# smithlabcode/epievo

Measured on AMD Instinct MI355X. Metric: site-branch path resamples/sec at n=1e6, 4-leaf tree, higher is better.
Workload: dtype f64

## Files before the change

epievo_amd/csrc/epv_abi.hip:

```cpp
#include <hip/hip_runtime.h>

#include <algorithm>
#include <chrono>
#include <cmath>
#include <cstdio>
#include <cstdlib>
#include <cstring>
#include <string>
#include <new>
#include <vector>

#include "epievo_mi355x.h"
#include "epv_device.h"
#include "epv_plan.h"

#define EPV_API extern "C" __attribute__((visibility("default")))

#include "epv_kernels.h"
#include "epv_math.h"
#include "epv_pavg.h"
#include "epv_bevents.h"
#include "epv_mixing.h"
#include "epv_wstat.h"
#include "epv_epochs.h"
// ... 1508 lines not shown
  auto raise = [](int kib, auto... kernels) {
    ((void)hipFuncSetAttribute(reinterpret_cast<const void *>(kernels), hipFuncAttributeMaxDynamicSharedMemorySize, kib * 1024), ...);
  };
  raise(128, p3_kernel(1u), p3_kernel(2u), p3_leaf_kernel(1u), p3_leaf_kernel(2u));
  raise(160, p2_kernel(false), p2_kernel(true), p2_leaf_kernel(false), p2_leaf_kernel(true));
  for (uint32_t nn = 0; nn <= EPV_P2_SMALL_MAX; ++nn) raise(160, fused_kernel(nn, false), fused_kernel(nn, true), fused_leaf_kernel(nn));
  for (int v = 0; v < 4; ++v)
    raise(160, v1_kernel<>(v & 1, v & 2), v1_kernel<leaf_arg_t>(v & 1, v & 2), v1_kernel<leaf_arg_t, leaf_arg_t>(v & 1, v & 2));
}

struct PhaseArgs {
  uint32_t colour, seed_lo, seed_hi, sweep;
  uint64_t first, last, own_lo, own_hi;
  uint64_t s0;
  uint64_t threads, blocks;
};

int launch_fused(epv_ctx *c, const PhasePlan &P, const PhaseArgs &a) {
  const PlanV2 &v = c->shapes.v2;
  const int frc = ensure_fused_buffers(c);
  if (frc) return frc;
  const unsigned pb = (unsigned)((a.threads + v.fused_lanes - 1u) / v.fused_lanes);
  if (pb > c->fused_waves) return fail(c, EPV_ERR_STATE, "fused phase: launch larger than its lists");
  EpvFused F = c->F;
  F.meta_cache = P.meta_cache ? 1u : 0u;
  F.lanes = v.fused_lanes;
  F.grouped_rounds = 4u;
  F.topo = 0u;
  for (uint32_t node = 1; node < P.small_nn; ++node)
    F.topo |= (c->subtree[node] == 1u ? 1u << node : 0u) | (c->parent[node] << (8u + 3u * node));
  F.giveups = c->d_counters + EPV_CNT_WORDS;
  if (P.unobs || P.evidence)
    hipLaunchKernelGGL(fused_leaf_kernel(P.small_nn), dim3(pb), dim3(64), v.lds, c->stream, c->S, a.colour, a.seed_lo,
                       a.seed_hi, a.sweep, a.first, a.last, a.own_lo, a.own_hi, v.pool, 0u, 0u, c->d_counters, (double *)nullptr,
                       c->d_segtab, F, (leaf_arg_t)c->d_evidence, (leaf_arg_t)c->d_unobs);
  else
  hipLaunchKernelGGL(fused_kernel(P.small_nn, P.direct), dim3(pb), dim3(64), v.lds, c->stream, c->S, a.colour, a.seed_lo,
                     a.seed_hi, a.sweep, a.first, a.last, a.own_lo, a.own_hi, v.pool, 0u, 0u, c->d_counters, (double *)nullptr,
                     c->d_segtab, F);
  return EPV_OK;
}

template <class... Leaf>
void launch_v1(epv_ctx *c, const PhasePlan &P, const PhaseArgs &a, Leaf... leaf) {
  const PlanV1 &v = c->shapes.v1;
  hipLaunchKernelGGL(v1_kernel<Leaf...>(P.gpool, P.refq), dim3((unsigned)a.blocks), dim3(v.threads), v.lds, c->stream, c->S,
                     a.colour, a.seed_lo, a.seed_hi, a.sweep, a.first, a.last, v.pool_entries, c->d_counters,
                     P.gpool ? c->d_gpool : (double *)nullptr, leaf...);
}
int launch_propose(epv_ctx *c, const PhasePlan &P, const PhaseArgs &a, uint32_t list_mode) {
  if (P.propose == EPV_PLAN_V3) {
    const PlanV3 &v = c->shapes.v3;
    const int rc = ensure_slab(c, &c->d_gpool3, &c->gpool3_cap, v.slab_need);
    if (rc) return rc;
    if (P.unobs || P.evidence)
      hipLaunchKernelGGL(p3_leaf_kernel(P.p3_words), dim3((unsigned)((a.threads + 255u) / 256u)), dim3(256), v.lds, c->stream,
                         c->S, a.colour, a.seed_lo, a.seed_hi, a.sweep, a.first, a.last, a.own_lo, a.own_hi, v.list_cap, v.qrows,
                         v.n_up, v.depth, list_mode - 1u, c->d_counters, c->d_gpool3, c->d_segtab, c->d_nodetab, c->d_slabflags,
                         v.slots, (leaf_arg_t)c->d_evidence, (leaf_arg_t)c->d_unobs);
    else
    hipLaunchKernelGGL(p3_kernel(P.p3_words), dim3((unsigned)((a.threads + 255u) / 256u)), dim3(256), v.lds, c->stream, c->S,
                       a.colour, a.seed_lo, a.seed_hi, a.sweep, a.first, a.last, a.own_lo, a.own_hi, v.list_cap, v.qrows,
                       v.n_up, v.depth, list_mode - 1u, c->d_counters, c->d_gpool3, c->d_segtab, c->d_nodetab, c->d_slabflags,
                       v.slots);
    ++c->phase_parity;
  } else if (P.propose == EPV_PLAN_V2) {
    const PlanV2 &v = c->shapes.v2;
    const bool seg = P.jumps == EPV_PLAN_JUMPS_SEGMENTS;
    if (seg) { const int rc = ensure_seg_buffers(c); if (rc) return rc; }
    if (P.unobs || P.evidence)
      hipLaunchKernelGGL(p2_leaf_kernel(seg), dim3((unsigned)((a.threads + 63u) / 64u)), dim3(64), v.lds, c->stream, c->S,
                         a.colour, a.seed_lo, a.seed_hi, a.sweep, a.first, a.last, a.own_lo, a.own_hi, v.pool, 0u, list_mode - 1u,
                         c->d_counters, (double *)nullptr, c->d_segtab, EpvFused{}, (leaf_arg_t)c->d_evidence,
                         (leaf_arg_t)c->d_unobs);
    else
    hipLaunchKernelGGL(p2_kernel(seg), dim3((unsigned)((a.threads + 63u) / 64u)), dim3(64), v.lds, c->stream, c->S, a.colour,
                       a.seed_lo, a.seed_hi, a.sweep, a.first, a.last, a.own_lo, a.own_hi, v.pool, 0u, list_mode - 1u,
                       c->d_counters, (double *)nullptr, c->d_segtab, EpvFused{});
    ++c->phase_parity;
  } else {
    if (P.gpool) { const int rc = ensure_slab(c, &c->d_gpool, &c->gpool_cap, c->shapes.v1.slab_need); if (rc) return rc; }
    if (P.evidence) launch_v1(c, P, a, (leaf_arg_t)c->d_evidence, (leaf_arg_t)c->d_unobs);
    else if (P.unobs) launch_v1(c, P, a, (leaf_arg_t)c->d_unobs);
    else launch_v1(c, P, a);
  }
  return EPV_OK;
}

void launch_jumps(epv_ctx *c, const PhasePlan &P, const PhaseArgs &a) {
  const size_t lds = const_lds_bytes(c->S.N);
  unsigned long long *giveups = c->d_counters + EPV_CNT_WORDS;
// ... 1624 lines not shown

EPV_API int epv_get_counters(epv_ctx *c, epv_counters *out) {
  if (!c || !out) return EPV_ERR_ARG;
  HIP_TRY(c, hipSetDevice(c->device));
  unsigned long long cnt[EPV_CNT_N];
  int rc = read_counters(c, cnt);
  if (rc) return rc;
  out->n_overflow = cnt[EPV_CNT_OVERFLOW];
  out->n_coop_tasks = cnt[EPV_CNT_COOP];
  out->n_sweeps = c->n_sweeps;
  out->n_search_finished = cnt[EPV_CNT_SEARCH_FINISHED];
  return EPV_OK;
}

#ifdef EPV_P2_PROFILE
EPV_API int epv_debug_p2_profile(unsigned long long *out) {
  std::vector<unsigned long long> rows(16u * EPV_P2_PROF_ROWS);
  if (hipMemcpyFromSymbol(rows.data(), HIP_SYMBOL(epv_p2_prof), rows.size() * sizeof(unsigned long long)) != hipSuccess) return 1;
  for (int q = 0; q < 16; ++q) out[q] = 0;
  for (size_t r = 0; r < EPV_P2_PROF_ROWS; ++r)
    for (int q = 0; q < 16; ++q) out[q] += rows[16u * r + q];
  return 0;
}
#endif

EPV_API int epv_set_timing(epv_ctx *c, int enabled) {
  if (!c) return EPV_ERR_ARG;
  c->timing_every = enabled > 0 ? (uint32_t)enabled : 0u;
  c->timing_seen = 0;
  c->timing = false;
  return EPV_OK;
}

EPV_API int epv_kernel_time_ms(epv_ctx *c, double *avg_ms, uint64_t *n_launches) {
  if (!c || !avg_ms || !n_launches) return EPV_ERR_ARG;
  HIP_TRY(c, hipSetDevice(c->device));
  HIP_TRY(c, hipStreamSynchronize(c->stream));
  int rc = drain_timing(c);
  if (rc) return rc;
  *n_launches = c->timed_launches;
  *avg_ms = c->timed_launches ? c->timed_ms / (double)c->timed_launches : 0.0;
  c->timed_ms = 0.0;
  c->timed_launches = 0;
  return EPV_OK;
}

// ... 842 lines not shown
```

epievo_amd/csrc/epv_plan.h:

```cpp
#ifndef EPV_PLAN_H
#define EPV_PLAN_H

#include <algorithm>
#include <cmath>
#include <cstdlib>
#include <vector>

#include "epv_device.h"

struct EpvKnobs {
  bool propose_v1 = false;
  int propose_v3 = -1;
  int seg_jumps = -1;
  int fused_phase = -1;
  bool small_tree = true;
  uint32_t fused_lanes = 0;
  bool force_lds_pool = false, force_global_pool = false;
  bool p3_min_list = false;
  int p3_slab_pool = 1;
  int accept_v3 = -1;
  bool accept_no_cache = false;
};

template <class Lookup>
// ... 70 lines not shown
  const uint32_t N = in.N, B = N - 1u, C = in.C;
  const uint64_t worst = (uint64_t)B * (2u * C + 2u);
  const size_t fixed = const_lds_bytes(N) + (((size_t)N * 64u * 4u + 15u) & ~(size_t)15u);
  if (fixed > 150u * 1024u) return false;
  const uint64_t typical = (uint64_t)(64.0 * B * (2.0 * in.kbar + 2.0) * 1.3) + 32u;
  const uint64_t max_fit = fixed + 16u < 160u * 1024u ? (160u * 1024u - fixed) / 16u : 0u;
  const uint64_t want = std::max<uint64_t>(worst, typical);
  const bool lds_ok = want <= max_fit && (fixed + std::min(want, max_fit) * 16u) * 8u <= 160u * 1024u;
  const bool use_lds = knobs.force_global_pool ? false : knobs.force_lds_pool ? want <= max_fit : lds_ok;
  if (use_lds) {
    const uint64_t pool = std::min(want, max_fit);
    v.pool_entries = (uint32_t)pool;
    v.lds = fixed + (size_t)pool * 16u;
  } else {
    const uint64_t blocks = (epv_phase_cap(in.n_sites) + 63u) / 64u;
    v.slab_need = blocks * worst * 128u;
    v.gpool = true;
    v.pool_entries = (uint32_t)worst;
    v.lds = fixed;
  }
  return true;
}

inline bool plan_p2(const PlanInput &in, const EpvKnobs &knobs, PlanV2 &v) {
  const uint32_t N = in.N, B = N - 1u, C = in.C;
  const uint64_t phase_cap = epv_phase_cap(in.n_sites);
  const size_t shared = const_lds_bytes(N) + (size_t)B * 4u * 6u * 8u;
  const size_t per_wave_fixed = ((((size_t)N * 64u + 1u) / 2u + 1u) & ~(size_t)1u) * 8u +
                                ((3u * 64u + 2u) * (size_t)B * sizeof(epv_meta_t) + 15u) / 16u * 16u;
  const size_t fixed = shared + per_wave_fixed;
  const uint64_t worst_rec = (uint64_t)B * (2u * C + 2u), worst_heavy = (uint64_t)B * (2u * C + 1u);
  uint32_t f_lanes = knobs.fused_lanes ? knobs.fused_lanes : 64u;
  if (!knobs.fused_lanes)
    while (f_lanes > 16u && (phase_cap + f_lanes / 2u - 1u) / (f_lanes / 2u) <= 2048u) f_lanes /= 2u;
  const uint64_t phase_waves = (phase_cap + 63u) / 64u;
  const uint64_t f_bytes = (phase_cap + f_lanes - 1u) / f_lanes *
                           (epv_fused_seg_cap(B, C) * (sizeof(EpvSegTask) + sizeof(EpvSegOut)) + epv_fused_bt_cap(B) * 12u);
  const bool fused = !knobs.propose_v1 && 2u * C + 1u <= 64u && f_bytes <= (4ull << 30) &&
                     (knobs.fused_phase < 0 ? phase_waves <= FUSED_MAX_WAVES : knobs.fused_phase != 0);
  const uint64_t hrec = (fused || seg_jumps_on(knobs, in.kbar)) ? EPV_HREC : EPV_HREC_SHORT;
  const uint64_t worst_dbl = 2u * worst_rec + hrec * worst_heavy;
  const double lam = 2.0 * in.kbar;
  uint32_t n_internal = 0;
  for (uint32_t node = 1; node < N; ++node) n_internal += in.subtree[node] != 1u;
  const double rec_per_lane = B * (1.0 + lam) + n_internal;
  const uint64_t typical_dbl = (uint64_t)(64.0 * (2.0 * rec_per_lane + (double)hrec * B * heavy_per_branch(lam)) * P2_MARGIN) + 64u;
  const uint64_t max_fit = fixed + 64u < 160u * 1024u ? (160u * 1024u - fixed) / 8u : 0u;
  uint64_t want = std::max(worst_dbl, typical_dbl);
  if (fused) want = std::max<uint64_t>(want, std::max<uint64_t>(EPV_COOP_BYTES / 8u, 992u + 48u * (uint64_t)B));
  const bool lds_ok = want <= max_fit && (fixed + want * 8u) * 5u <= 160u * 1024u;
  const bool use_lds = knobs.force_global_pool ? false : knobs.force_lds_pool ? want <= max_fit : lds_ok;
  if (fixed > 150u * 1024u) return false;
  v.planned = use_lds;
  v.fused = fused && use_lds;
  v.fused_lanes = f_lanes;
  v.pool = use_lds ? (uint32_t)((want + 1u) & ~(uint64_t)1u) : 0u;
  v.lds = fixed + (size_t)v.pool * 8u;
  return true;
}

inline PlanV3 plan_p3(const PlanInput &in, const EpvKnobs &knobs, const PlanV2 &v2) {
  const uint32_t N = in.N, B = N - 1u, C = in.C;
  if (knobs.propose_v3 == 0 || knobs.propose_v1 || N > 128u || N < 2u) return {};
  if (knobs.propose_v3 < 0 && v2.planned) return {};
// ... 145 lines not shown
```

epievo_amd/csrc/epv_propose2.h:

```cpp
#ifndef EPV_PROPOSE2_H
#define EPV_PROPOSE2_H

struct EpvSegRec {
  double P00, P11;
  double PT00, PT10;
  double nb0, nb1;
  double u_end, u_first;
  double len;
  uint64_t info;
};

EPV_DEV void epv_seg_matrices(double len, double r0, double r1, double out[6]) {
  const double denom = r0 + r1;
  const double h = 1.0 / epv_exp(len * (r0 + r1));
  out[0] = (r0 * h + r1) / denom;
  out[1] = (r0 + r1 * h) / denom;
  const double h2 = epv_exp(-len * (r0 + r1));
  out[2] = gtp(r0, r1, h2, denom, 0u, 0u);
  out[3] = gtp(r0, r1, h2, denom, 1u, 0u);
#if defined(__HIP_DEVICE_COMPILE__)
  out[4] = nojump_bound(len * r0);
  out[5] = nojump_bound(len * r1);
#else
  out[4] = 0.0;
  out[5] = 0.0;
#endif
}

__global__ void epv_segtab_kernel(EpvDev S, double *tab) {
  const uint32_t t = blockIdx.x * blockDim.x + threadIdx.x;
  if (t >= S.B * 4u) return;
  const uint32_t b = t >> 2, li = (t >> 1) & 1u, ri = t & 1u;
  const double *rates = reinterpret_cast<const double *>(S.model);
  const uint32_t trip0 = 4u * li + ri;
// ... 64 lines not shown
  uint32_t grouped_rounds;
  uint32_t topo;
  unsigned long long *giveups;
};

template <bool SEG, bool FUSED, int NN = 0, bool DIRECT = false, class... Leaf>
__global__ __launch_bounds__(256, EPV_PROPOSE2_WAVES) void epv_mh_propose2_kernel(
    EpvDev S, uint32_t colour, uint32_t seed_lo, uint32_t seed_hi, uint32_t sweep, uint64_t first,
    uint64_t last, uint64_t own_first, uint64_t own_last, uint32_t pool_dbl, uint32_t list_cap,
    uint32_t parity, unsigned long long *counters, double *gpool, const double *segtab, EpvFused F, Leaf... leaf_args) {
  constexpr bool LEAF = sizeof...(Leaf) != 0;
  static_assert(sizeof...(Leaf) == (LEAF ? 2u : 0u), "the table and the mask come together");
  [[maybe_unused]] EpvLeafSrc LS{nullptr, nullptr};
  if constexpr (LEAF) { LS.table = epv_first_arg(leaf_args...); LS.mask = epv_second_arg(leaf_args...); }
  static_assert(!FUSED || SEG, "the fused phase emits segments");
  static_assert(!DIRECT || FUSED, "the direct body is the fused phase's");
  static_assert(!LEAF || !DIRECT, "the fused direct bodies have no leaf variant");
  constexpr bool SMALL = NN > 0;
  static_assert(!SMALL || (FUSED && NN >= 2 && NN <= EPV_P2_SMALL_MAX), "the small-tree body is the fused phase's");
  constexpr int NNA = SMALL ? NN : 1;
  constexpr int NBA = SMALL ? NN - 1 : 1;
  const uint32_t NNODE = SMALL ? (uint32_t)NN : S.N;
  extern __shared__ __attribute__((aligned(16))) double s_mem[];
  constexpr uint32_t HREC = SEG ? EPV_HREC : EPV_HREC_SHORT, LEN_AT = HREC - 2u, INFO_AT = HREC - 1u;
#ifdef EPV_P2_PROFILE
  unsigned long long t_acc_[16] = {0, 0, 0, 0, 0, 0, 0, 0, 0, 0, 0, 0, 0, 0, 0, 0};
  unsigned long long t_prev_ = __builtin_readcyclecounter();
#endif
  const uint32_t B = SMALL ? (uint32_t)NN - 1u : S.B;
  const uint32_t const_dbl = (20u + NNODE + 1u) & ~1u;
  const uint32_t tab_dbl = B * 4u * EPV_SEGTAB_DBL;
  const uint32_t regA_dbl = ((NNODE * 64u + 1u) / 2u + 1u) & ~1u;
  const uint32_t mc_dbl = ((3u * 64u + 2u) * B * (uint32_t)sizeof(epv_meta_t) + 15u) / 16u * 2u;
  const uint32_t wave_id = threadIdx.x >> 6;
  const uint32_t my_shard = (blockIdx.x * (blockDim.x >> 6) + wave_id) & (EPV_SHARDS - 1u);
  const uint32_t wave_dbl = regA_dbl + mc_dbl + ((pool_dbl + 1u) & ~1u);
  double *s_const = s_mem;
  double *s_tab = s_mem + const_dbl;
  double *s_wave = s_mem + const_dbl + tab_dbl + (size_t)wave_id * wave_dbl;
  uint32_t *regA = reinterpret_cast<uint32_t *>(s_wave);
  epv_meta_t *s_meta = reinterpret_cast<epv_meta_t *>(s_wave + regA_dbl);
  epv_meta_t *s_edge = s_meta + 3u * B * 64u;
  const int lane = epv_lane();
  double *pool = s_wave + regA_dbl + mc_dbl;
  const uint64_t gfirst = S.g0 + first;
  const uint64_t s0 = first + ((colour + 3u - (uint32_t)(gfirst % 3u)) % 3u);
  const uint32_t lpw = FUSED ? F.lanes : 64u;
// ... 198 lines not shown
      }
      __builtin_amdgcn_fence(__ATOMIC_SEQ_CST, "wavefront");
      __builtin_amdgcn_wave_barrier();
    } else if (run && heavy) {
      uint32_t hcur = hbase;
      for (uint32_t node = 1u; node < NNODE; ++node) {
        const uint32_t b = node - 1u;
        const uint32_t K = (s_meta[(0u * B + b) * 64u + lane] & EPV_NJ_MASK) + (s_meta[(1u * B + b) * 64u + lane] & EPV_NJ_MASK) + 1u;
        if (K < 2u) continue;
        merge_branch((uint32_t)lane, node, hcur, jbaseL, jbaseR);
        hcur += K;
      }
    }
    __builtin_amdgcn_fence(__ATOMIC_SEQ_CST, "wavefront");
    __builtin_amdgcn_wave_barrier();

    P2_MARK(2);
    for (uint32_t i = (uint32_t)lane; i < totH; i += 64u) {
      double *rec = list + (size_t)i * HREC;
      const double len = rec[LEN_AT];
      const uint64_t info = epv_d2u(rec[INFO_AT]);
      const uint32_t trip0 = (uint32_t)info & 7u, owner = (uint32_t)(info >> 3) & 63u;
      const uint32_t node = (uint32_t)(info >> 9) & 4095u, k = (uint32_t)(info >> 21);
      double m[6];
      epv_seg_matrices(len, s_rates[trip0], s_rates[trip0 | 2u], m);
      const epv_block2 blk = epv_keyed_block<!FUSED>(seed_lo, seed_hi, gsite_lane0 + 3u * owner, sweep, node, k, 0u, 0u);
#pragma unroll
      for (int q = 0; q < 6; ++q) rec[q] = m[q];
      rec[6] = blk.d0;
      rec[7] = blk.d1;
    }
    __builtin_amdgcn_fence(__ATOMIC_SEQ_CST, "wavefront");
    __builtin_amdgcn_wave_barrier();

    P2_MARK(3);
    bool ident = true;
    if (run) {
      uint32_t off = need_rec, hcur = hbase + heavy;
#pragma unroll 1
      for (uint32_t node = NNODE - 1u; node >= 1u; --node) {
        const uint32_t b = node - 1u;
        [[maybe_unused]] uint32_t leaf_word = 0u;
        if constexpr (LEAF) {
          if (SMALL ? EPV_TOPO_LEAF(node) != 0u : S.subtree[node] == 1u) leaf_word = epv_leaf_word(LS, node, site);
        }
        const uint32_t mL = s_meta[(0u * B + b) * 64u + lane], mR = s_meta[(1u * B + b) * 64u + lane];
        const uint32_t K = (mL & EPV_NJ_MASK) + (mR & EPV_NJ_MASK) + 1u;
        const uint32_t sub = SMALL ? 2u - EPV_TOPO_LEAF(node) : S.subtree[node];
        off -= K + (LEAF || sub != 1u ? 1u : 0u);
        double n0 = 1.0, n1 = 1.0;
        if (sub == 1u) {
          const uint32_t mM = s_meta[(2u * B + b) * 64u + lane];
          const uint32_t leaf_state = (mM >> EPV_INIT_SHIFT) ^ (mM & 1u);
// ... 26 lines not shown
          const double *t = s_tab + (b * 4u + 2u * (mL >> EPV_INIT_SHIFT) + (mR >> EPV_INIT_SHIFT)) * EPV_SEGTAB_DBL;
          const double P00 = t[0], P11 = t[1];
          const double P01 = 1.0 - P00, P10 = 1.0 - P11;
          double *rec = my + (size_t)off * RS;
          rec[0] = P00 * n0 + P01 * n1;
          rec[1] = P10 * n0 + P11 * n1;
        } else {
          hcur -= K;
          for (uint32_t kk = K; kk-- > 0u;) {
            const double *hr = list + (size_t)(hcur + kk) * HREC;
            const double P00 = hr[0], P11 = hr[1];
            const double P01 = 1.0 - P00, P10 = 1.0 - P11;
            const double a = P00 * n0 + P01 * n1;
            const double c = P10 * n0 + P11 * n1;
            double *rec = my + (size_t)(off + kk) * RS;
            rec[0] = a; rec[1] = c;
            n0 = a; n1 = c;
          }
        }
      }
    }

    P2_MARK(4);
    unsigned long long dirty = 0ull, multi = 0ull, deep = 0ull;
    const uint32_t root_state = run ? (uint32_t)(s_meta[(2u * B) * 64u + lane] >> EPV_INIT_SHIFT) : 0u;
    uint32_t hcur = hbase;
    if constexpr (SMALL) {
      if (run) {
#pragma unroll
        for (int node = 1; node < NNA; ++node) r_node[node] = regA[(uint32_t)node * 64u + lane];
#pragma unroll
        for (int node = 1; node < NNA; ++node) {
          const int b = node - 1;
          const uint32_t K = EPV_RW_K(r_w[b]);
          const uint32_t off = r_node[node];
          uint32_t start_state = root_state;
#pragma unroll
          for (int p = 1; p < node; ++p)
            if (EPV_TOPO_PARENT(node) == (uint32_t)p) start_state = r_node[p] >> 31;
          const bool leaf = EPV_TOPO_LEAF(node);
          const uint32_t mM = EPV_RW_META(r_w[b]);
          uint32_t prev = start_state;
          bool clean = true;
          unsigned long long word = 0ull, w64 = 0ull;
          double pk0 = my[(size_t)off * RS], pk1 = my[(size_t)off * RS + 1u];
          for (uint32_t k = 0; k < K; ++k) {
            const bool last_seg = (k + 1u == K);
            double nxt0, nxt1;
            if (!LEAF && last_seg && leaf) {
              const uint32_t leaf_state = (mM >> EPV_INIT_SHIFT) ^ (mM & 1u);
              nxt0 = leaf_state ? 0.0 : 1.0;
              nxt1 = leaf_state ? 1.0 : 0.0;
            } else {
              nxt0 = my[(size_t)(off + k + 1u) * RS];
              nxt1 = my[(size_t)(off + k + 1u) * RS + 1u];
            }
            double PT0, nb, u_end, u_first;
            if (K == 1u) {
              const double *t = s_tab + ((uint32_t)b * 4u + EPV_RW_TAB(r_w[b])) * EPV_SEGTAB_DBL;
              PT0 = prev ? t[3] : t[2];
              nb = prev ? t[5] : t[4];
              const epv_block2 blk = epv_keyed_block<!FUSED>(seed_lo, seed_hi, gsite, sweep, (uint32_t)node, 0u, 0u, 0u);
              u_end = blk.d0; u_first = blk.d1;
            } else {
              const double *hr = list + (size_t)(hcur + k) * HREC;
              PT0 = prev ? hr[3] : hr[2];
              nb = prev ? hr[5] : hr[4];
              u_end = hr[6]; u_first = hr[7];
            }
            const double p0 = PT0 * nxt0 / (prev ? pk1 : pk0);
            const uint32_t sampled = (u_end > p0) ? 1u : 0u;
            const bool seg_clean = (sampled == prev) && (1.0 - u_first < nb);
            clean = clean && seg_clean;
            word |= (unsigned long long)sampled << (k & 63u);
            if (k < 64u) w64 = word;
            prev = sampled;
            pk0 = nxt0; pk1 = nxt1;
          }
          const uint32_t hrec0 = hcur;
          if (K >= 2u) hcur += K;
          r_node[node] = off | (prev << 31) | (clean ? 0u : 1u << 30) | (K >= 2u ? hrec0 << 14 : 0u);
          regA[node * 64u + lane] = r_node[node];
          if (!clean && K >= 2u) list[(size_t)hrec0 * HREC + 6u] = epv_u2d(w64);
          s_meta[(2u * B + (uint32_t)b) * 64u + lane] = (epv_meta_t)(start_state << EPV_INIT_SHIFT);
          ident = ident && clean && mM == (start_state << EPV_INIT_SHIFT);
        }
      }
    } else
    for (uint32_t node = 1u; node < S.N; ++node) {
      const uint32_t b = node - 1u;
      uint32_t nds = 0, Kb = 0, st_b = 0, end_b = 0, hrec0 = 0, trip_b = 0;
      unsigned long long w64 = 0ull;
      bool dirty_b = false;
      if (run) {
        const uint32_t mL = s_meta[(0u * B + b) * 64u + lane], mR = s_meta[(1u * B + b) * 64u + lane];
        const uint32_t K = (mL & EPV_NJ_MASK) + (mR & EPV_NJ_MASK) + 1u;
        const uint32_t off = regA[node * 64u + lane];
        const uint32_t par = S.parent[node];
        const uint32_t start_state = (par == 0u) ? root_state : (regA[par * 64u + lane] >> 31);
        const bool leaf = S.subtree[node] == 1u;
        const uint32_t mM = s_meta[(2u * B + b) * 64u + lane];
        uint32_t prev = start_state;
        bool clean = true;
        unsigned long long word = 0ull;
        uint64_t *states = S.prop_states + ((uint64_t)b * S.phase_cap + tid) * S.W;
        double pk0 = my[(size_t)off * RS], pk1 = my[(size_t)off * RS + 1u];
        for (uint32_t k = 0; k < K; ++k) {
          const bool last_seg = (k + 1u == K);
          double nxt0, nxt1;
          if (!LEAF && last_seg && leaf) {
            const uint32_t leaf_state = (mM >> EPV_INIT_SHIFT) ^ (mM & 1u);
            nxt0 = leaf_state ? 0.0 : 1.0;
            nxt1 = leaf_state ? 1.0 : 0.0;
          } else {
            nxt0 = my[(size_t)(off + k + 1u) * RS];
            nxt1 = my[(size_t)(off + k + 1u) * RS + 1u];
          }
          double PT0, nb, u_end, u_first;
          if (K == 1u) {
            const double *t = s_tab + (b * 4u + 2u * (mL >> EPV_INIT_SHIFT) + (mR >> EPV_INIT_SHIFT)) * EPV_SEGTAB_DBL;
            PT0 = prev ? t[3] : t[2];
            nb = prev ? t[5] : t[4];
            const epv_block2 blk = epv_keyed_block<!FUSED>(seed_lo, seed_hi, gsite, sweep, node, 0u, 0u, 0u);
            u_end = blk.d0; u_first = blk.d1;
          } else {
            const double *hr = list + (size_t)(hcur + k) * HREC;
            PT0 = prev ? hr[3] : hr[2];
            nb = prev ? hr[5] : hr[4];
            u_end = hr[6]; u_first = hr[7];
          }
          const double p0 = PT0 * nxt0 / (prev ? pk1 : pk0);
          const uint32_t sampled = (u_end > p0) ? 1u : 0u;
          const bool seg_clean = (sampled == prev) && (1.0 - u_first < nb);
          clean = clean && seg_clean;
          nds += seg_clean ? 0u : 1u;
          word |= (unsigned long long)sampled << (k & 63u);
          if (k < 64u) w64 = word;
          if (!FUSED && (k & 63u) == 63u) { states[k >> 6] = word; word = 0ull; }
          prev = sampled;
          pk0 = nxt0; pk1 = nxt1;
        }
        hrec0 = hcur;
        if (K >= 2u) hcur += K;
        if (!FUSED && (K & 63u) && !clean) states[(K - 1u) >> 6] = word;
        if (FUSED) {
          regA[node * 64u + lane] = off | (prev << 31) | (clean ? 0u : 1u << 30) | (K >= 2u ? hrec0 << 14 : 0u);
          if (!clean && K >= 2u) list[(size_t)hrec0 * HREC + 6u] = epv_u2d(w64);
        } else
          regA[node * 64u + lane] = off | (prev << 31);
        if (FUSED) s_meta[(2u * B + b) * 64u + lane] = (epv_meta_t)(start_state << EPV_INIT_SHIFT);
        ident = ident && clean && mM == (start_state << EPV_INIT_SHIFT);
        dirty_b = !clean;
        Kb = K; st_b = start_state; end_b = prev;
        trip_b = 4u * (mL >> EPV_INIT_SHIFT) + (mR >> EPV_INIT_SHIFT);
      }
      bool old_list = dirty_b;
      if (SEG && !FUSED) {
        const bool cand = dirty_b && Kb <= 64u;
        const uint32_t wS = cand ? nds : 0u, wB = cand ? 1u : 0u;
        const uint32_t inclS = wave_incl_scan_u32(wS), inclB = wave_incl_scan_u32(wB);
        const uint32_t totS = epv_bcast(inclS, 63), totB = epv_bcast(inclB, 63);
        if (totB) {
          const uint32_t shard = my_shard;
          uint32_t bS, bB;
          if (FUSED) {
            bS = f_nseg; bB = f_nbt;
            f_nseg += totS; f_nbt += totB;
          } else {
            unsigned long long base = 0ull;
            if (lane == 0)
// ... 118 lines not shown
        for (uint32_t node = 1u; node < S.N; ++node)
          if ((regA[node * 64u + lane] >> 30) & 1u) plist[at++] = (uint32_t)lane | (node << 6);
      }
      __builtin_amdgcn_fence(__ATOMIC_SEQ_CST, "wavefront");
      __builtin_amdgcn_wave_barrier();
      const uint64_t site_lane0 = site - 3u * (uint64_t)lane;
      EpvSegTask *segs_w = F.segs + f_wave * F.seg_cap;
      unsigned long long *btl = F.bt + f_wave * F.bt_cap;
      uint32_t *bfl = F.bfirst + f_wave * F.bt_cap;
      for (uint32_t p0 = 0; p0 < totP; p0 += 64u) {
        const uint32_t pidx = p0 + (uint32_t)lane;
        const bool act = pidx < totP;
        const uint32_t pr = act ? plist[pidx] : 0u;
        const uint32_t owner = pr & 63u, node = act ? pr >> 6 : 1u, b = node - 1u;
        const uint32_t selM_o = (uint32_t)__shfl((int)selM, (int)owner);
        const uint32_t ra = regA[node * 64u + owner];
        const uint32_t end_b = ra >> 31, hrec0 = (ra >> 14) & 0x3fffu;
        const uint32_t st_b = (uint32_t)(s_meta[(2u * B + b) * 64u + owner] >> EPV_INIT_SHIFT);
        const uint32_t mL = s_meta[(0u * B + b) * 64u + owner], mR = s_meta[(1u * B + b) * 64u + owner];
        const uint32_t Kb = (mL & EPV_NJ_MASK) + (mR & EPV_NJ_MASK) + 1u;
        unsigned long long w64 = end_b, dmask = 1ull;
        uint32_t nds = act ? 1u : 0u;
        if (act && Kb >= 2u) {
          w64 = epv_d2u(list[(size_t)hrec0 * HREC + 6u]);
          dmask = 0ull;
          nds = 0u;
          uint32_t prev = st_b;
          for (uint32_t k = 0; k < Kb; ++k) {
            const double *hr = list + (size_t)(hrec0 + k) * HREC;
            const uint32_t sampled = (uint32_t)(w64 >> k) & 1u;
            const bool seg_clean = (sampled == prev) && (1.0 - hr[7] < (prev ? hr[5] : hr[4]));
            if (!seg_clean) { dmask |= 1ull << k; ++nds; }
            prev = sampled;
          }
        }
        const uint32_t inclS = wave_incl_scan_u32(nds);
        const uint32_t totS = epv_bcast(inclS, 63);
        if (act) {
          const uint64_t osite = site_lane0 + 3u * (uint64_t)owner;
          const uint64_t i0 = (uint64_t)f_nseg + (inclS - nds), j0 = (uint64_t)f_nbt + (uint32_t)lane;
          btl[j0] = osite | ((unsigned long long)b << 40) | ((unsigned long long)nds << 52) | ((unsigned long long)end_b << 59) |
                    ((unsigned long long)st_b << 60) | ((unsigned long long)(selM_o ^ 1u) << 61);
          bfl[j0] = (uint32_t)i0;
          uint32_t prev = st_b;
          double tp = 0.0;
          uint64_t at = i0;
          for (uint32_t k = 0; k < Kb; ++k) {
            const uint32_t sampled = (uint32_t)(w64 >> k) & 1u;
            double len;
            uint32_t trip0;
            if (Kb == 1u) {
              len = s_blen[node];
              trip0 = 4u * (mL >> EPV_INIT_SHIFT) + (mR >> EPV_INIT_SHIFT);
            } else {
              const double *hr = list + (size_t)(hrec0 + k) * HREC;
              len = hr[LEN_AT];
              trip0 = (uint32_t)epv_d2u(hr[INFO_AT]) & 7u;
// ... 179 lines not shown
```

epievo_amd/csrc/host/epv_host_abi.cpp:

```cpp
#include <algorithm>
#include <cstring>
#include <stdexcept>
#include <string>
#include <vector>

#include "epv_model.hpp"
#include "epv_sim.hpp"
#include "epv_io.hpp"
#include "epv_domains.hpp"
#include "epv_turnover.hpp"
#include "epv_corr.hpp"
#include "epv_dmaps.hpp"
#include "epv_epochs.hpp"
#include "epv_indep.hpp"
#include "epv_forward.hpp"
#include "epievo_mi355x.h"
#include "../epv_plan.h"

namespace {
thread_local std::string g_err;
void put_model(const epv::Model &m, double *rates, double *T, double *baseline) {
  for (int i = 0; i < 8; ++i) rates[i] = m.rates[i];
  for (int i = 0; i < 4; ++i) { T[i] = m.T[i]; baseline[i] = m.baseline[i]; }
}
// ... 619 lines not shown
  for (size_t i = 0; i < es->node_names.size(); ++i) joined += (i ? "\n" : "") + es->node_names[i];
  return joined;
}
EPVH_API void epvh_epoch_stats_dims(void *h, uint64_t *n_samples, uint64_t *n_epochs, uint64_t *n_branches,
                                    uint64_t *names_len) {
  const epv::EpochStats *es = (const epv::EpochStats *)h;
  *names_len = joined_names(es).size() + 1u;
  *n_samples = es->n_samples;
  *n_epochs = es->n_epochs;
  *n_branches = es->node_names.size();
}
EPVH_API void epvh_epoch_stats_copy(void *h, char *names, int names_len, double *branch_len, int *scale_exp,
                                    uint64_t *closed, double *start, double *factor) {
  const epv::EpochStats *es = (const epv::EpochStats *)h;
  put_text(joined_names(es), names, names_len);
  std::copy(es->branch_len.begin(), es->branch_len.end(), branch_len);
  std::copy(es->scale_exp.begin(), es->scale_exp.end(), scale_exp);
  std::copy(es->closed.begin(), es->closed.end(), closed);
  std::copy(es->start.begin(), es->start.end(), start);
  std::copy(es->factor.begin(), es->factor.end(), factor);
}
EPVH_API void epvh_epoch_stats_free(void *h) { delete (epv::EpochStats *)h; }

EPVH_API int epvh_phase_plan(int n_nodes, const uint32_t *parent_ids, const uint32_t *subtree_sizes, uint64_t n_sites,
                             uint32_t capacity, double kbar, uint32_t options, uint64_t unobs_cells,
                             uint64_t evidence_cells, const char *const *knobs, int n_knobs, uint32_t *word) {
  if (n_nodes < 2 || n_nodes > 4095 || !parent_ids || !subtree_sizes || !word || n_knobs < 0 || (n_knobs && !knobs)) {
    g_err = "bad tree";
    return 1;
  }
  for (int i = 1; i < n_nodes; ++i)
    if (parent_ids[i] >= (uint32_t)i || subtree_sizes[i] < 1 || i + subtree_sizes[i] > (uint32_t)n_nodes) {
      g_err = "tree arrays are not a valid pre-order tree";
      return 1;
    }
  if (n_sites < 3 || capacity < 1 || capacity > EPV_MAX_CAP || !(kbar >= 0.0)) {
    g_err = "bad paths: at least 3 sites, a capacity of 1 .. 2047, a mean jump count >= 0";
    return 1;
  }
  const EpvKnobs k = read_knobs([&](const char *name) -> const char * {
    const size_t len = std::strlen(name);
    for (int i = 0; i < n_knobs; ++i)
      if (knobs[i] && !std::strncmp(knobs[i], name, len) && knobs[i][len] == '=') return knobs[i] + len + 1;
    return nullptr;
  });
  const PhaseShapes shapes = plan_shapes({(uint32_t)n_nodes, parent_ids, subtree_sizes, capacity, n_sites, kbar}, k);
  if (shapes.error) {
    g_err = shapes.error;
    return 1;
  }
  *word = phase_plan(shapes, k, options, unobs_cells, evidence_cells, (uint32_t)n_nodes - 1u, kbar).word();
  return 0;
}
```

epievo_amd/host.py:

```python
import ctypes as C
import os

import numpy as np

from . import _build

_lib = None


def lib():
    global _lib
    if _lib is None:
        path = _build.HOST_SO
        if not os.path.exists(path):
            _build.build_host()
        L = C.CDLL(path)
        dp, u8p, u32p, u64p = (C.POINTER(C.c_double), C.POINTER(C.c_uint8),
                               C.POINTER(C.c_uint32), C.POINTER(C.c_uint64))
        L.epvh_last_error.restype = C.c_char_p
        L.epvh_model_read.argtypes = [C.c_char_p, C.c_int, dp, dp, dp]
        L.epvh_rate_scaling_factor.argtypes = [dp]
        L.epvh_rate_scaling_factor.restype = C.c_double
        L.epvh_m_step.argtypes = [C.c_int, C.c_int, dp, dp, dp, dp, dp, dp, dp, C.c_char_p, C.c_int]
        L.epvh_simulate.argtypes = [dp, dp, C.c_int, u32p, dp, C.c_uint64, C.c_uint64]
# ... 90 lines not shown
        L.epvh_domain_maps_dims.argtypes = [C.c_void_p, u64p]
        L.epvh_domain_maps_dims.restype = None
        L.epvh_domain_maps_copy.argtypes = [C.c_void_p, C.c_char_p, C.c_int, u32p, u64p]
        L.epvh_domain_maps_copy.restype = None
        L.epvh_domain_maps_free.argtypes = [C.c_void_p]
        L.epvh_domain_maps_free.restype = None
        u64p_, u32 = C.POINTER(C.c_uint64), C.c_uint32
        L.epvh_epoch_edges.argtypes = [C.c_uint64, u32, u64p_]
        L.epvh_epoch_edges.restype = None
        L.epvh_epoch_close.argtypes = [u64p_, u64p_, u32, u32, u64p_]
        L.epvh_epoch_counts_to_stats.argtypes = [u64p_, C.POINTER(C.c_int), u32, u32, C.c_uint64, dp, dp]
        L.epvh_write_epoch_stats.argtypes = [C.c_char_p, C.c_char_p, C.c_int, u32, dp, C.POINTER(C.c_int), u64p_, u64p_,
                                             C.c_uint64, dp]
        L.epvh_read_epoch_stats.argtypes = [C.c_char_p]
        L.epvh_read_epoch_stats.restype = C.c_void_p
        L.epvh_epoch_stats_dims.argtypes = [C.c_void_p, u64p_, u64p_, u64p_, u64p_]
        L.epvh_epoch_stats_dims.restype = None
        L.epvh_epoch_stats_copy.argtypes = [C.c_void_p, C.c_char_p, C.c_int, dp, C.POINTER(C.c_int), u64p_, dp, dp]
        L.epvh_epoch_stats_copy.restype = None
        L.epvh_epoch_stats_free.argtypes = [C.c_void_p]
        L.epvh_epoch_stats_free.restype = None
        L.epvh_phase_plan.argtypes = [C.c_int, u32p, u32p, C.c_uint64, u32, C.c_double, u32, C.c_uint64, C.c_uint64,
                                      C.POINTER(C.c_char_p), C.c_int, C.POINTER(u32)]
        _lib = L
    return _lib


def _p(a, t):
    return a.ctypes.data_as(C.POINTER(t))


class Model:

    def __init__(self, rates, T, baseline):
        self.rates = np.ascontiguousarray(rates, dtype=np.float64)
        self.T = np.ascontiguousarray(T, dtype=np.float64)
        self.baseline = np.ascontiguousarray(baseline, dtype=np.float64)

    @staticmethod
    def read(param_file, scale=True):
        rates, T, bl = np.zeros(8), np.zeros(4), np.zeros(4)
        if lib().epvh_model_read(param_file.encode(), int(scale), _p(rates, C.c_double),
                                 _p(T, C.c_double), _p(bl, C.c_double)):
            raise RuntimeError(lib().epvh_last_error().decode())
        return Model(rates, T, bl)

# ... 67 lines not shown
        init = self.init.reshape(B, n)[:, lo:hi]
        offs = self.offsets[:-1].reshape(B, n)[:, lo:hi]
        pieces = [self.jumps[int(offs[b, 0]):int(offs[b, -1] + cnt[b, -1])] for b in range(B)]
        new_off = np.zeros(B * (hi - lo) + 1, np.uint64)
        new_off[1:] = np.cumsum(cnt.reshape(-1))
        return FlatPaths(hi - lo, self.n_nodes, init.reshape(-1).copy(), new_off,
                         np.concatenate(pieces) if pieces else np.zeros(0))


PLAN_PROPOSE = ("V1", "V2", "V3", "fused")
PLAN_JUMPS = ("fused", "segments", "jumps_all", "jumps")
PLAN_ACCEPT = ("fused", "accept3", "accept_cache", "accept_no_cache")


def plan_fields(w):
    return dict(word=w, propose=PLAN_PROPOSE[w & 3], gpool=bool(w >> 2 & 1), refq=bool(w >> 3 & 1),
                small_nn=w >> 4 & 15, p3_words=w >> 8 & 3, p3_slab_pool=bool(w >> 10 & 1),
                jumps=PLAN_JUMPS[w >> 12 & 3], accept=PLAN_ACCEPT[w >> 14 & 3], listed=bool(w >> 16 & 1),
                unobs=bool(w >> 17 & 1), evidence=bool(w >> 18 & 1), direct=bool(w >> 23 & 1),
                fused_lanes=(1 << (w >> 20 & 7)) if (w & 3) == 3 else 0)


def phase_plan(tree, n_sites, capacity, kbar, options=0, unobs_cells=0, evidence_cells=0, knobs={}):
    names = [("%s=%s" % kv).encode() for kv in knobs.items()]
    arr = (C.c_char_p * max(len(names), 1))(*names)
    w = C.c_uint32(0)
    if lib().epvh_phase_plan(tree.n_nodes, _p(tree.parent_ids, C.c_uint32), _p(tree.subtree_sizes, C.c_uint32),
                             int(n_sites), int(capacity), float(kbar), int(options), int(unobs_cells),
                             int(evidence_cells), arr, len(names), C.byref(w)):
        raise RuntimeError(lib().epvh_last_error().decode())
    return plan_fields(int(w.value))


def simulate(model, tree, n_sites, seed):
    h = lib().epvh_simulate(_p(model.rates, C.c_double), _p(model.T, C.c_double), tree.n_nodes,
                            _p(tree.parent_ids, C.c_uint32), _p(tree.branches, C.c_double),
                            int(n_sites), int(seed))
    if not h:
        raise RuntimeError(lib().epvh_last_error().decode())
    return FlatPaths._from_handle(h)


def read_paths(path_file, max_nodes=4096):
    buf = C.create_string_buffer(64 * max_nodes)
    tt = np.zeros(max_nodes)
    h = lib().epvh_read_paths(path_file.encode(), buf, len(buf), _p(tt, C.c_double), max_nodes)
    if not h:
        raise RuntimeError(lib().epvh_last_error().decode())
    fp = FlatPaths._from_handle(h)
    return fp, buf.value.decode().split("\n"), tt[:fp.n_nodes].copy()


def write_paths(path_file, node_names, tot_times, fp):
    tt = np.ascontiguousarray(tot_times, dtype=np.float64)
# ... 792 lines not shown
```

Before: 20.29 billion.

## Shrink fused heavy-segment records and cache the dirty mask instead of recomputing it

In the fused kernel, heavy-segment records now use the short record size. The prune pass stores only the two pruning probabilities, and a separate pass after pruning overwrites those slots with the sampling matrices and random draws. The forward pass also records a per-branch dirty-segment mask next to the state word, so the later pass reads it and takes a popcount instead of re-scanning every segment. The goal is a smaller LDS/global record pool, which may allow higher occupancy, and less redundant work. The cost is an extra pass with wave barriers, plus new checks that the pool can hold one lane's worst case.

```diff
diff --git a/epievo_amd/csrc/epv_abi.hip b/epievo_amd/csrc/epv_abi.hip
--- a/epievo_amd/csrc/epv_abi.hip
+++ b/epievo_amd/csrc/epv_abi.hip
@@ -1554,6 +1554,8 @@
   if (frc) return frc;
   const unsigned pb = (unsigned)((a.threads + v.fused_lanes - 1u) / v.fused_lanes);
   if (pb > c->fused_waves) return fail(c, EPV_ERR_STATE, "fused phase: launch larger than its lists");
+  if (v.pool < p2_worst_dbl(c->S.B, c->S.C, p2_hrec(true, true)))
+    return fail(c, EPV_ERR_STATE, "fused phase: the record pool is below one lane's worst case");
   EpvFused F = c->F;
   F.meta_cache = P.meta_cache ? 1u : 0u;
   F.lanes = v.fused_lanes;
@@ -1599,6 +1601,8 @@
   } else if (P.propose == EPV_PLAN_V2) {
     const PlanV2 &v = c->shapes.v2;
     const bool seg = P.jumps == EPV_PLAN_JUMPS_SEGMENTS;
+    if (v.pool < p2_worst_dbl(c->S.B, c->S.C, p2_hrec(false, seg)))
+      return fail(c, EPV_ERR_STATE, "second proposal kernel: the record pool is below one lane's worst case");
     if (seg) { const int rc = ensure_seg_buffers(c); if (rc) return rc; }
     if (P.unobs || P.evidence)
       hipLaunchKernelGGL(p2_leaf_kernel(seg), dim3((unsigned)((a.threads + 63u) / 64u)), dim3(64), v.lds, c->stream, c->S,
@@ -3269,6 +3273,14 @@
     for (int q = 0; q < 16; ++q) out[q] += rows[16u * r + q];
   return 0;
 }
+EPV_API int epv_debug_p2_occupancy(epv_ctx *c, int *blocks, unsigned long long *lds) {
+  if (!c || !blocks || !lds || !c->have_paths) return EPV_ERR_ARG;
+  const PhasePlan P = phase_plan(c);
+  if (P.propose != EPV_PLAN_FUSED) return EPV_ERR_STATE;
+  *lds = c->shapes.v2.lds;
+  return hipOccupancyMaxActiveBlocksPerMultiprocessor(blocks, reinterpret_cast<const void *>(fused_kernel(P.small_nn, P.direct)), 64,
+                                                      c->shapes.v2.lds) == hipSuccess ? EPV_OK : EPV_ERR_HIP;
+}
 #endif
 
 EPV_API int epv_set_timing(epv_ctx *c, int enabled) {
diff --git a/epievo_amd/csrc/epv_plan.h b/epievo_amd/csrc/epv_plan.h
--- a/epievo_amd/csrc/epv_plan.h
+++ b/epievo_amd/csrc/epv_plan.h
@@ -116,6 +116,12 @@
   return true;
 }
 
+inline uint32_t p2_hrec(bool fused_body, bool seg) { return !fused_body && seg ? EPV_HREC : EPV_HREC_SHORT; }
+inline uint32_t p2_hrec_max(const EpvKnobs &knobs, double kbar) { return p2_hrec(false, seg_jumps_on(knobs, kbar)); }
+inline uint64_t p2_worst_dbl(uint32_t B, uint32_t C, uint32_t hrec) {
+  return 2u * (uint64_t)B * (2u * C + 2u) + (uint64_t)hrec * B * (2u * C + 1u);
+}
+
 inline bool plan_p2(const PlanInput &in, const EpvKnobs &knobs, PlanV2 &v) {
   const uint32_t N = in.N, B = N - 1u, C = in.C;
   const uint64_t phase_cap = epv_phase_cap(in.n_sites);
@@ -123,7 +129,6 @@
   const size_t per_wave_fixed = ((((size_t)N * 64u + 1u) / 2u + 1u) & ~(size_t)1u) * 8u +
                                 ((3u * 64u + 2u) * (size_t)B * sizeof(epv_meta_t) + 15u) / 16u * 16u;
   const size_t fixed = shared + per_wave_fixed;
-  const uint64_t worst_rec = (uint64_t)B * (2u * C + 2u), worst_heavy = (uint64_t)B * (2u * C + 1u);
   uint32_t f_lanes = knobs.fused_lanes ? knobs.fused_lanes : 64u;
   if (!knobs.fused_lanes)
     while (f_lanes > 16u && (phase_cap + f_lanes / 2u - 1u) / (f_lanes / 2u) <= 2048u) f_lanes /= 2u;
@@ -132,8 +137,8 @@
                            (epv_fused_seg_cap(B, C) * (sizeof(EpvSegTask) + sizeof(EpvSegOut)) + epv_fused_bt_cap(B) * 12u);
   const bool fused = !knobs.propose_v1 && 2u * C + 1u <= 64u && f_bytes <= (4ull << 30) &&
                      (knobs.fused_phase < 0 ? phase_waves <= FUSED_MAX_WAVES : knobs.fused_phase != 0);
-  const uint64_t hrec = (fused || seg_jumps_on(knobs, in.kbar)) ? EPV_HREC : EPV_HREC_SHORT;
-  const uint64_t worst_dbl = 2u * worst_rec + hrec * worst_heavy;
+  const uint64_t hrec = p2_hrec_max(knobs, in.kbar);
+  const uint64_t worst_dbl = p2_worst_dbl(B, C, (uint32_t)hrec);
   const double lam = 2.0 * in.kbar;
   uint32_t n_internal = 0;
   for (uint32_t node = 1; node < N; ++node) n_internal += in.subtree[node] != 1u;
diff --git a/epievo_amd/csrc/epv_propose2.h b/epievo_amd/csrc/epv_propose2.h
--- a/epievo_amd/csrc/epv_propose2.h
+++ b/epievo_amd/csrc/epv_propose2.h
@@ -10,6 +10,25 @@
   uint64_t info;
 };
 
+EPV_DEV void epv_seg_prune_matrix(double len, double r0, double r1, double out[2]) {
+  const double denom = r0 + r1;
+  const double h = 1.0 / epv_exp(len * (r0 + r1));
+  out[0] = (r0 * h + r1) / denom;
+  out[1] = (r0 + r1 * h) / denom;
+}
+EPV_DEV void epv_seg_sample_matrices(double len, double r0, double r1, double out[4]) {
+  const double denom = r0 + r1;
+  const double h2 = epv_exp(-len * (r0 + r1));
+  out[0] = gtp(r0, r1, h2, denom, 0u, 0u);
+  out[1] = gtp(r0, r1, h2, denom, 1u, 0u);
+#if defined(__HIP_DEVICE_COMPILE__)
+  out[2] = nojump_bound(len * r0);
+  out[3] = nojump_bound(len * r1);
+#else
+  out[2] = 0.0;
+  out[3] = 0.0;
+#endif
+}
 EPV_DEV void epv_seg_matrices(double len, double r0, double r1, double out[6]) {
   const double denom = r0 + r1;
   const double h = 1.0 / epv_exp(len * (r0 + r1));
@@ -120,7 +139,9 @@
   constexpr int NBA = SMALL ? NN - 1 : 1;
   const uint32_t NNODE = SMALL ? (uint32_t)NN : S.N;
   extern __shared__ __attribute__((aligned(16))) double s_mem[];
-  constexpr uint32_t HREC = SEG ? EPV_HREC : EPV_HREC_SHORT, LEN_AT = HREC - 2u, INFO_AT = HREC - 1u;
+  constexpr uint32_t HREC = (SEG && !FUSED) ? EPV_HREC : EPV_HREC_SHORT, LEN_AT = HREC - 2u, INFO_AT = HREC - 1u;
+  constexpr uint32_t F_PT = FUSED ? 0u : 2u, F_NB = FUSED ? 2u : 4u, F_UEND = FUSED ? 4u : 6u, F_UFIRST = FUSED ? 5u : 7u;
+  [[maybe_unused]] constexpr uint32_t F_W64 = F_UEND, F_DMASK = F_UFIRST;
 #ifdef EPV_P2_PROFILE
   unsigned long long t_acc_[16] = {0, 0, 0, 0, 0, 0, 0, 0, 0, 0, 0, 0, 0, 0, 0, 0};
   unsigned long long t_prev_ = __builtin_readcyclecounter();
@@ -365,13 +386,20 @@
       const uint64_t info = epv_d2u(rec[INFO_AT]);
       const uint32_t trip0 = (uint32_t)info & 7u, owner = (uint32_t)(info >> 3) & 63u;
       const uint32_t node = (uint32_t)(info >> 9) & 4095u, k = (uint32_t)(info >> 21);
-      double m[6];
-      epv_seg_matrices(len, s_rates[trip0], s_rates[trip0 | 2u], m);
-      const epv_block2 blk = epv_keyed_block<!FUSED>(seed_lo, seed_hi, gsite_lane0 + 3u * owner, sweep, node, k, 0u, 0u);
-#pragma unroll
-      for (int q = 0; q < 6; ++q) rec[q] = m[q];
-      rec[6] = blk.d0;
-      rec[7] = blk.d1;
+      if constexpr (FUSED) {
+        double m[2];
+        epv_seg_prune_matrix(len, s_rates[trip0], s_rates[trip0 | 2u], m);
+        rec[0] = m[0];
+        rec[1] = m[1];
+      } else {
+        double m[6];
+        epv_seg_matrices(len, s_rates[trip0], s_rates[trip0 | 2u], m);
+        const epv_block2 blk = epv_keyed_block<!FUSED>(seed_lo, seed_hi, gsite_lane0 + 3u * owner, sweep, node, k, 0u, 0u);
+#pragma unroll
+        for (int q = 0; q < 6; ++q) rec[q] = m[q];
+        rec[6] = blk.d0;
+        rec[7] = blk.d1;
+      }
     }
     __builtin_amdgcn_fence(__ATOMIC_SEQ_CST, "wavefront");
     __builtin_amdgcn_wave_barrier();
@@ -444,6 +472,29 @@
     }
 
     P2_MARK(4);
+    if constexpr (FUSED) {
+      __builtin_amdgcn_fence(__ATOMIC_SEQ_CST, "wavefront");
+      __builtin_amdgcn_wave_barrier();
+      for (uint32_t i = (uint32_t)lane; i < totH; i += 64u) {
+        double *rec = list + (size_t)i * HREC;
+        const double len = rec[LEN_AT];
+        const uint64_t info = epv_d2u(rec[INFO_AT]);
+        const uint32_t trip0 = (uint32_t)info & 7u, owner = (uint32_t)(info >> 3) & 63u;
+        const uint32_t node = (uint32_t)(info >> 9) & 4095u, k = (uint32_t)(info >> 21);
+        double m[4];
+        epv_seg_sample_matrices(len, s_rates[trip0], s_rates[trip0 | 2u], m);
+        const epv_block2 blk = epv_keyed_block<!FUSED>(seed_lo, seed_hi, gsite_lane0 + 3u * owner, sweep, node, k, 0u, 0u);
+        rec[F_PT] = m[0];
+        rec[F_PT + 1u] = m[1];
+        rec[F_NB] = m[2];
+        rec[F_NB + 1u] = m[3];
+        rec[F_UEND] = blk.d0;
+        rec[F_UFIRST] = blk.d1;
+      }
+      __builtin_amdgcn_fence(__ATOMIC_SEQ_CST, "wavefront");
+      __builtin_amdgcn_wave_barrier();
+      P2_MARK(10);
+    }
     unsigned long long dirty = 0ull, multi = 0ull, deep = 0ull;
     const uint32_t root_state = run ? (uint32_t)(s_meta[(2u * B) * 64u + lane] >> EPV_INIT_SHIFT) : 0u;
     uint32_t hcur = hbase;
@@ -464,7 +515,7 @@
           const uint32_t mM = EPV_RW_META(r_w[b]);
           uint32_t prev = start_state;
           bool clean = true;
-          unsigned long long word = 0ull, w64 = 0ull;
+          unsigned long long word = 0ull, w64 = 0ull, dmask = 0ull;
           double pk0 = my[(size_t)off * RS], pk1 = my[(size_t)off * RS + 1u];
           for (uint32_t k = 0; k < K; ++k) {
             const bool last_seg = (k + 1u == K);
@@ -486,14 +537,15 @@
               u_end = blk.d0; u_first = blk.d1;
             } else {
               const double *hr = list + (size_t)(hcur + k) * HREC;
-              PT0 = prev ? hr[3] : hr[2];
-              nb = prev ? hr[5] : hr[4];
-              u_end = hr[6]; u_first = hr[7];
+              PT0 = prev ? hr[F_PT + 1u] : hr[F_PT];
+              nb = prev ? hr[F_NB + 1u] : hr[F_NB];
+              u_end = hr[F_UEND]; u_first = hr[F_UFIRST];
             }
             const double p0 = PT0 * nxt0 / (prev ? pk1 : pk0);
             const uint32_t sampled = (u_end > p0) ? 1u : 0u;
             const bool seg_clean = (sampled == prev) && (1.0 - u_first < nb);
             clean = clean && seg_clean;
+            if (!seg_clean) dmask |= 1ull << (k & 63u);
             word |= (unsigned long long)sampled << (k & 63u);
             if (k < 64u) w64 = word;
             prev = sampled;
@@ -503,7 +555,10 @@
           if (K >= 2u) hcur += K;
           r_node[node] = off | (prev << 31) | (clean ? 0u : 1u << 30) | (K >= 2u ? hrec0 << 14 : 0u);
           regA[node * 64u + lane] = r_node[node];
-          if (!clean && K >= 2u) list[(size_t)hrec0 * HREC + 6u] = epv_u2d(w64);
+          if (!clean && K >= 2u) {
+            list[(size_t)hrec0 * HREC + F_W64] = epv_u2d(w64);
+            list[(size_t)hrec0 * HREC + F_DMASK] = epv_u2d(dmask);
+          }
           s_meta[(2u * B + (uint32_t)b) * 64u + lane] = (epv_meta_t)(start_state << EPV_INIT_SHIFT);
           ident = ident && clean && mM == (start_state << EPV_INIT_SHIFT);
         }
@@ -512,7 +567,7 @@
     for (uint32_t node = 1u; node < S.N; ++node) {
       const uint32_t b = node - 1u;
       uint32_t nds = 0, Kb = 0, st_b = 0, end_b = 0, hrec0 = 0, trip_b = 0;
-      unsigned long long w64 = 0ull;
+      unsigned long long w64 = 0ull, dmask = 0ull;
       bool dirty_b = false;
       if (run) {
         const uint32_t mL = s_meta[(0u * B + b) * 64u + lane], mR = s_meta[(1u * B + b) * 64u + lane];
@@ -547,15 +602,16 @@
             u_end = blk.d0; u_first = blk.d1;
           } else {
             const double *hr = list + (size_t)(hcur + k) * HREC;
-            PT0 = prev ? hr[3] : hr[2];
-            nb = prev ? hr[5] : hr[4];
-            u_end = hr[6]; u_first = hr[7];
+            PT0 = prev ? hr[F_PT + 1u] : hr[F_PT];
+            nb = prev ? hr[F_NB + 1u] : hr[F_NB];
+            u_end = hr[F_UEND]; u_first = hr[F_UFIRST];
           }
           const double p0 = PT0 * nxt0 / (prev ? pk1 : pk0);
           const uint32_t sampled = (u_end > p0) ? 1u : 0u;
           const bool seg_clean = (sampled == prev) && (1.0 - u_first < nb);
           clean = clean && seg_clean;
           nds += seg_clean ? 0u : 1u;
+          if (FUSED && !seg_clean) dmask |= 1ull << (k & 63u);
           word |= (unsigned long long)sampled << (k & 63u);
           if (k < 64u) w64 = word;
           if (!FUSED && (k & 63u) == 63u) { states[k >> 6] = word; word = 0ull; }
@@ -567,7 +623,10 @@
         if (!FUSED && (K & 63u) && !clean) states[(K - 1u) >> 6] = word;
         if (FUSED) {
           regA[node * 64u + lane] = off | (prev << 31) | (clean ? 0u : 1u << 30) | (K >= 2u ? hrec0 << 14 : 0u);
-          if (!clean && K >= 2u) list[(size_t)hrec0 * HREC + 6u] = epv_u2d(w64);
+          if (!clean && K >= 2u) {
+            list[(size_t)hrec0 * HREC + F_W64] = epv_u2d(w64);
+            list[(size_t)hrec0 * HREC + F_DMASK] = epv_u2d(dmask);
+          }
         } else
           regA[node * 64u + lane] = off | (prev << 31);
         if (FUSED) s_meta[(2u * B + b) * 64u + lane] = (epv_meta_t)(start_state << EPV_INIT_SHIFT);
@@ -732,17 +791,9 @@
         unsigned long long w64 = end_b, dmask = 1ull;
         uint32_t nds = act ? 1u : 0u;
         if (act && Kb >= 2u) {
-          w64 = epv_d2u(list[(size_t)hrec0 * HREC + 6u]);
-          dmask = 0ull;
-          nds = 0u;
-          uint32_t prev = st_b;
-          for (uint32_t k = 0; k < Kb; ++k) {
-            const double *hr = list + (size_t)(hrec0 + k) * HREC;
-            const uint32_t sampled = (uint32_t)(w64 >> k) & 1u;
-            const bool seg_clean = (sampled == prev) && (1.0 - hr[7] < (prev ? hr[5] : hr[4]));
-            if (!seg_clean) { dmask |= 1ull << k; ++nds; }
-            prev = sampled;
-          }
+          w64 = epv_d2u(list[(size_t)hrec0 * HREC + F_W64]);
+          dmask = epv_d2u(list[(size_t)hrec0 * HREC + F_DMASK]);
+          nds = (uint32_t)__popcll(dmask);
         }
         const uint32_t inclS = wave_incl_scan_u32(nds);
         const uint32_t totS = epv_bcast(inclS, 63);
diff --git a/epievo_amd/csrc/host/epv_host_abi.cpp b/epievo_amd/csrc/host/epv_host_abi.cpp
--- a/epievo_amd/csrc/host/epv_host_abi.cpp
+++ b/epievo_amd/csrc/host/epv_host_abi.cpp
@@ -665,9 +665,10 @@
 }
 EPVH_API void epvh_epoch_stats_free(void *h) { delete (epv::EpochStats *)h; }
 
-EPVH_API int epvh_phase_plan(int n_nodes, const uint32_t *parent_ids, const uint32_t *subtree_sizes, uint64_t n_sites,
-                             uint32_t capacity, double kbar, uint32_t options, uint64_t unobs_cells,
-                             uint64_t evidence_cells, const char *const *knobs, int n_knobs, uint32_t *word) {
+EPVH_API int epvh_phase_plan2(int n_nodes, const uint32_t *parent_ids, const uint32_t *subtree_sizes, uint64_t n_sites,
+                              uint32_t capacity, double kbar, uint32_t options, uint64_t unobs_cells,
+                              uint64_t evidence_cells, const char *const *knobs, int n_knobs, uint32_t *word,
+                              uint64_t p2[5]) {
   if (n_nodes < 2 || n_nodes > 4095 || !parent_ids || !subtree_sizes || !word || n_knobs < 0 || (n_knobs && !knobs)) {
     g_err = "bad tree";
     return 1;
@@ -693,5 +694,15 @@
     return 1;
   }
   *word = phase_plan(shapes, k, options, unobs_cells, evidence_cells, (uint32_t)n_nodes - 1u, kbar).word();
+  if (p2) {
+    const PlanV2 &v = shapes.v2;
+    p2[0] = v.planned ? 1u : 0u; p2[1] = v.fused ? 1u : 0u; p2[2] = v.pool; p2[3] = v.lds; p2[4] = v.fused_lanes;
+  }
   return 0;
 }
+EPVH_API int epvh_phase_plan(int n_nodes, const uint32_t *parent_ids, const uint32_t *subtree_sizes, uint64_t n_sites,
+                             uint32_t capacity, double kbar, uint32_t options, uint64_t unobs_cells,
+                             uint64_t evidence_cells, const char *const *knobs, int n_knobs, uint32_t *word) {
+  return epvh_phase_plan2(n_nodes, parent_ids, subtree_sizes, n_sites, capacity, kbar, options, unobs_cells, evidence_cells,
+                          knobs, n_knobs, word, nullptr);
+}
diff --git a/epievo_amd/host.py b/epievo_amd/host.py
--- a/epievo_amd/host.py
+++ b/epievo_amd/host.py
@@ -136,6 +136,7 @@
         L.epvh_epoch_stats_free.restype = None
         L.epvh_phase_plan.argtypes = [C.c_int, u32p, u32p, C.c_uint64, u32, C.c_double, u32, C.c_uint64, C.c_uint64,
                                       C.POINTER(C.c_char_p), C.c_int, C.POINTER(u32)]
+        L.epvh_phase_plan2.argtypes = L.epvh_phase_plan.argtypes + [u64p_]
         _lib = L
     return _lib
 
@@ -249,14 +250,20 @@
 
 
 def phase_plan(tree, n_sites, capacity, kbar, options=0, unobs_cells=0, evidence_cells=0, knobs={}):
+    return phase_plan_p2(tree, n_sites, capacity, kbar, options, unobs_cells, evidence_cells, knobs)[0]
+
+
+def phase_plan_p2(tree, n_sites, capacity, kbar, options=0, unobs_cells=0, evidence_cells=0, knobs={}):
     names = [("%s=%s" % kv).encode() for kv in knobs.items()]
     arr = (C.c_char_p * max(len(names), 1))(*names)
     w = C.c_uint32(0)
-    if lib().epvh_phase_plan(tree.n_nodes, _p(tree.parent_ids, C.c_uint32), _p(tree.subtree_sizes, C.c_uint32),
-                             int(n_sites), int(capacity), float(kbar), int(options), int(unobs_cells),
-                             int(evidence_cells), arr, len(names), C.byref(w)):
-        raise RuntimeError(lib().epvh_last_error().decode())
-    return plan_fields(int(w.value))
+    p2 = (C.c_uint64 * 5)()
+    if lib().epvh_phase_plan2(tree.n_nodes, _p(tree.parent_ids, C.c_uint32), _p(tree.subtree_sizes, C.c_uint32),
+                              int(n_sites), int(capacity), float(kbar), int(options), int(unobs_cells),
+                              int(evidence_cells), arr, len(names), C.byref(w), p2):
+        raise RuntimeError(lib().epvh_last_error().decode())
+    return plan_fields(int(w.value)), dict(planned=bool(p2[0]), fused=bool(p2[1]), pool=int(p2[2]), lds=int(p2[3]),
+                                           fused_lanes=int(p2[4]))
 
 
 def simulate(model, tree, n_sites, seed):
```

Result: faster. 20.87 billion, median of 6 (+2.9%).
